# HKU-MedAI/WSI-HGNN

Measured on AMD Instinct MI355X. Metric: edges/s fwd+bwd HEATNet4, 10k-node/6-rel synth graph, 1->8 MI355X, higher is better.
Workload: dtype f32 (fp16x3 emulation: 2-way fp16 split scaled per row (Y = XW^T, dX) or per column (dW), 3 products - bf16x6 for small launches; fp32-class error)

## Files before the change

include/wsi_hgnn.h:

```cpp
#ifndef WSI_HGNN_H
#define WSI_HGNN_H

#include <stdint.h>

#ifdef __cplusplus
extern "C" {
#endif

#define WSI_OK        0
#define WSI_EINVAL  (-22)
#define WSI_ENOSYS  (-38)
#define WSI_EFAULT  (-14)
#define WSI_ENOMEM  (-12)

#define WSI_ABI_VERSION 26

int         wsi_abi_version(void);
const char* wsi_last_error(void);

typedef struct wsi_context wsi_context_t;
int  wsi_context_create(wsi_context_t** out);
void wsi_context_destroy(wsi_context_t* ctx);

#define WSI_ATTN_XCD_CONTIGUOUS 1
// ... 227 lines not shown
int wsi_gate_grad(const float* g, int64_t ldg, const float* a, int64_t lda, const float* b, int64_t ldb,
                  int32_t D, const int32_t* chunk_row, int32_t num_chunks, const int32_t* seg_chunk, int32_t num_segs,
                  const int32_t* seg_gate, const float* skip, int32_t n_gates, float* partial, float* g_skip, void* stream);

int wsi_pool_factors(const float* x, int64_t ldx, int32_t D, const float* w, int64_t ldw, int32_t T, int32_t H, int32_t Bg,
                     const int32_t* chunk_row, int32_t num_chunks, const int32_t* seg_chunk,
                     float* partial, float* hp, float* csum, float* x_mean, void* stream);
int wsi_pool_tmean(const float* tpart, int32_t T, int32_t S, int32_t D, int32_t H, const float* csum, const float* const* bv,
                   const float* scale, float* t_mean, void* stream);
int wsi_pool_bwd_prep(const float* g_pool, int32_t S, int32_t D, int32_t op, const float* counts, const float* z_mean, const float* h_mean,
                      const int32_t* seg_gate, const float* skip, int32_t n_gates, const int32_t* type_gate, int32_t T,
                      float* g_row, float* g_sum, float* g_skip, float* omg, void* stream);
int wsi_pool_bwd_bias(const float* gt_seg, int32_t T, int32_t S, int32_t D, int32_t H, const float* const* bv, const float* csum,
                      float* beta, float* gbv, void* stream);

int wsi_plan_assemble(const int64_t* desc, int32_t nsegs, int32_t total_blocks, void* stream);
int wsi_slot_fill(const int64_t* desc, int32_t nsegs, int32_t total_blocks, void* stream);

int wsi_layernorm_fwd(const float* x, int64_t ldx, int32_t n, int32_t D, float eps,
                      const float* gamma, const float* beta, const int32_t* row_param,
                      float* y, int64_t ldy, float* stats, void* stream);
int wsi_layernorm_bwd(const float* gy, int64_t ldgy, const float* x, int64_t ldx, int32_t n, int32_t D,
                      const float* gamma, const int32_t* row_param, const float* stats,
                      float* gx, int64_t ldgx, float* xhat_gy, int64_t ldp, void* stream);
int wsi_gelu_fwd(const float* x, float* y, int64_t n, void* stream);
int wsi_gelu_bwd(const float* x, const float* gy, float* gx, int64_t n, void* stream);
int wsi_spmm_sum(const float* x, int64_t ldx, int32_t n_out, int32_t D,
                 const int32_t* ptr, const int32_t* idx, const float* edge_w, const float* iscale, const float* oscale,
                 const float* bias, int32_t relu, const float* relu_ref, int64_t ldref,
                 float* out, int64_t ldo, void* stream);
// ... 173 lines not shown
```

wsi-hgnn_amd/csrc/heat_attn.hip:

```cpp
#include "common.h"
#include <math.h>
#include <stdlib.h>
#include <mutex>
#include <type_traits>
#include <new>

namespace wsi {

struct AttnGraph {
    const int32_t* node_seg;
    const int32_t* rowptr;
    const int32_t* src;
    const float* sim;
    const int32_t* order;
    int32_t num_nodes;
    int32_t heavy_n;
    int32_t pass;
    int32_t heavy_deg;
    int32_t xcd;
    uint32_t* absmax;
    const float* score_in;
    const int32_t* gt_row;
};

// ... 432 lines not shown
#pragma unroll
        for (int i = 0; i < V; ++i) {
            float x = 0.f;
#pragma unroll
            for (int pp = 0; pp < kWavesPerBlock; ++pp) x += sm_acc[(pp * V + i) * 64 + lane];
            gqa[i] = x;
        }
    }
    store_vec<V>(gq + (int64_t)w * ldgq + col, gqa);
    if (g.absmax) {
        const uint32_t b = wave_absmax_bits<V>(gqa);
        if (lane == 0) g.absmax[2 * (int64_t)w] = b;
    }
}

template <int V, int LPH, int U, bool POOL = false, bool KONLY = false>
__global__ __launch_bounds__(kBlock) void heat_attn_bwd_p3_kernel(
    const float* __restrict__ qtab, int64_t ldq, const float* __restrict__ g_t, int64_t ldgt,
    const int32_t* __restrict__ colptr, const int32_t* __restrict__ csc_eid, const int32_t* __restrict__ csc_dst,
    const float* __restrict__ inv_rd, const int32_t* __restrict__ order, int32_t num_nodes, int32_t xcd,
    const float* __restrict__ a, const float* __restrict__ gsc,
    float* __restrict__ gk, int64_t ldgk, float* __restrict__ gv, int64_t ldgv, uint32_t* __restrict__ absmax,
    const int32_t* __restrict__ gt_row, AttnPool pool) {
    constexpr int H = 64 / LPH;
    const int lane = threadIdx.x & 63;
    const int blk = xcd ? xcd_remap((int)blockIdx.x, (int)gridDim.x) : (int)blockIdx.x;
    int wave = blk * kWavesPerBlock + (int)(threadIdx.x >> 6);
    wave = __builtin_amdgcn_readfirstlane(wave);
    if (wave >= num_nodes) return;
    int u = order ? order[wave] : wave;
    u = __builtin_amdgcn_readfirstlane(u);
// ... 6 lines not shown
    float cb[POOL ? kPoolTypes : 1];
#pragma unroll
    for (int b = 0; b < (POOL ? kPoolTypes : 1); ++b) cb[b] = 0.f;

    const int j0 = colptr[u], j1 = colptr[u + 1];
    for (int j = j0; j < j1; j += U) {
        float qq[U][V], gt[U][V];
        float aa[U], gg[U];
        int bin[U];
#pragma unroll
        for (int x = 0; x < U; ++x) {
            if (j + x < j1) {
                const int eid = csc_eid[j + x];
                const int w = csc_dst[j + x];
                const int64_t o = (int64_t)eid * H + head;
                if constexpr (!KONLY) aa[x] = a[o] * inv_rd[w];
                gg[x] = gsc[o];
                load_vec<V>(qq[x], qtab + (int64_t)w * ldq + col);
                if constexpr (POOL) bin[x] = pool.ctab_ready ? -1 : pool.row_seg[w] / pool.segs_per_type;
                else if constexpr (!KONLY) load_vec<V>(gt[x], g_t + (int64_t)(gt_row ? gt_row[w] : w) * ldgt + col);
            }
        }
#pragma unroll
        for (int x = 0; x < U; ++x) {
            if (j + x < j1) {
#pragma unroll
                for (int i = 0; i < V; ++i) {
                    gka[i] = fmaf(gg[x], qq[x][i], gka[i]);
                    if constexpr (!POOL && !KONLY) gva[i] = fmaf(aa[x], gt[x][i], gva[i]);
                }
                if constexpr (POOL) {
#pragma unroll
                    for (int b = 0; b < kPoolTypes; ++b) cb[b] += (bin[x] == b) ? aa[x] : 0.f;
                }
            }
        }
    }
    store_vec<V>(gk + (int64_t)u * ldgk + col, gka);
    if constexpr (POOL) {
        const int su = pool.row_seg[u];
        const int tu = su / pool.segs_per_type, gu = su - tu * pool.segs_per_type;
        float racc[V];
        load_vec<V>(racc, pool.g_row + (int64_t)su * (V * 64) + col);
        const float om = pool.omg[tu];
#pragma unroll
        for (int i = 0; i < V; ++i) racc[i] *= om;
        const float* ybase = pool.y + (int64_t)tu * pool.num_segs * H * (V * 64);
#pragma unroll
        for (int b = 0; b < kPoolTypes; ++b) {
            if (b < pool.n_types) {
                if (pool.ctab_ready) cb[b] = pool.ctab[((int64_t)u * pool.n_types + b) * H + head];
                const float* yrow = ybase + (int64_t)(b * pool.segs_per_type + gu) * H * (V * 64) + col;
#pragma unroll
                for (int h = 0; h < H; ++h) {
                    const float c = __shfl(cb[b], h * LPH, 64);
                    float yv[V];
                    load_vec<V>(yv, yrow + h * (V * 64));
#pragma unroll
                    for (int i = 0; i < V; ++i) racc[i] = fmaf(c, yv[i], racc[i]);
                }
                if (!pool.ctab_ready && (lane % LPH) == 0) pool.ctab[((int64_t)u * pool.n_types + b) * H + head] = cb[b];
            }
        }
        store_vec<V>(pool.r_out + (int64_t)u * pool.ldr + col, racc);
        if (absmax) {
            const uint32_t bmax = wave_absmax_bits<V>(gka);
            if (lane == 0) absmax[2 * (int64_t)u + 1] = bmax;
        }
    } else if constexpr (KONLY) {
        if (absmax) {
            const uint32_t b = wave_absmax_bits<V>(gka);
            if (lane == 0) absmax[2 * (int64_t)u + 1] = max(b, absmax[2 * (int64_t)u + 1]);
        }
    } else {
        store_vec<V>(gv + (int64_t)u * ldgv + col, gva);
        if (absmax) {
            const uint32_t b = max(wave_absmax_bits<V>(gka), wave_absmax_bits<V>(gva));
            if (lane == 0) absmax[2 * (int64_t)u + 1] = b;
        }
// ... 538 lines not shown
        if (pflat || srcmajor) {}
        else if (ph) hipLaunchKernelGGL((heat_attn_bwd_p1_kernel<V, LPH, U, false, true>), dim3(blocks), dim3(kBlock), 0, st, tb, gl, g_t, ldgt, score_a, lse, ga, *pool);
        else hipLaunchKernelGGL((heat_attn_bwd_p1_kernel<V, LPH, U>), dim3(blocks), dim3(kBlock), 0, st, tb, gl, g_t, ldgt, score_a, lse, ga, AttnPool{});
        hipLaunchKernelGGL((heat_attn_bwd_p2_kernel<V, LPH, U>), dim3(blocks), dim3(kBlock), 0, st,
                           tb, gl, ew, eb, isd, (const float*)score_a, (const float*)ga, gsc, gea, gq, ldgq);
        hub_join(st, side);
    } else if (blocks > 0) {
        if (pflat || srcmajor) {}
        else if (ph) hipLaunchKernelGGL((heat_attn_bwd_p1_kernel<V, LPH, U, false, true>), dim3(blocks), dim3(kBlock), 0, st,
                                        tb, gd, g_t, ldgt, score_a, lse, ga, *pool);
        else hipLaunchKernelGGL((heat_attn_bwd_p1_kernel<V, LPH, U>), dim3(blocks), dim3(kBlock), 0, st,
                                tb, gd, g_t, ldgt, score_a, lse, ga, AttnPool{});
        hipLaunchKernelGGL((heat_attn_bwd_p2_kernel<V, LPH, U>), dim3(blocks), dim3(kBlock), 0, st,
                           tb, gd, ew, eb, isd, (const float*)score_a, (const float*)ga, gsc, gea, gq, ldgq);
    }
    if (sblocks > 0 && pool)
        hipLaunchKernelGGL((heat_attn_bwd_p3_kernel<V, LPH, U, true>), dim3(sblocks), dim3(kBlock), 0, st,
                           tb.q, tb.ldq, g_t, ldgt, colptr, csc_eid, csc_dst, inv_rd, order_src, num_src, gd.xcd,
                           (const float*)score_a, (const float*)gsc, gk, ldgk, gv, ldgv, gd.absmax, gd.gt_row, *pool);
    else if (sblocks > 0 && srcmajor) {
        constexpr int UC = U;
        auto pass_c = [&](auto uu) {
            hipLaunchKernelGGL((heat_attn_bwd_p3_kernel<V, LPH, decltype(uu)::value, false, true>), dim3(sblocks), dim3(kBlock), 0, st,
                               tb.q, tb.ldq, g_t, ldgt, colptr, csc_eid, csc_dst, inv_rd, order_src, num_src, gd.xcd,
                               (const float*)score_a, (const float*)gsc, gk, ldgk, gv, ldgv, gd.absmax, gd.gt_row, AttnPool{});
        };
#ifdef WSI_ABLATE
        const char* su = knob("WSI_ATTN_SRC_U");
        const int uc = su ? su[su[0] && su[1] ? 1 : 0] - '0' : UC;
        if (uc == 2) pass_c(std::integral_constant<int, 2>{});
        else if (uc == 4) pass_c(std::integral_constant<int, 4>{});
// ... 60 lines not shown
                                 int32_t num_nodes, int32_t num_src, int32_t num_edges, int32_t D, int32_t H,
                                 const int32_t* node_seg, const int32_t* rowptr, const int32_t* src, const float* sim,
                                 const int32_t* colptr, const int32_t* csc_eid, const int32_t* csc_dst,
                                 const float* inv_rd, const int32_t* order_dst, int32_t num_heavy, const int32_t* order_src, int32_t flags,
                                 const float* e_weight, const float* e_bias,
                                 const float* g_t, int64_t ldgt, const int32_t* g_t_row, const float* score, float* score_a, const float* lse,
                                 float* ga, float* gsc, float* gea, float* red_ws,
                                 float* gq, int64_t ldgq, float* gk, int64_t ldgk, float* gv, int64_t ldgv,
                                 float* g_e, uint32_t* g_absmax, const wsi_attn_pool_t* pool, wsi_context_t* ctx, void* stream) {
    if (num_nodes < 0 || num_src < 0 || num_edges < 0 || D <= 0 || H <= 0 || D % H != 0) { set_error("heat_attn_bwd: bad shape"); return WSI_EINVAL; }
    if (!q || !k || (!v && !(pool && (pool->h || pool->gtab))) || !node_seg || !rowptr || !colptr || !inv_rd || !e_weight || !e_bias || !g_t || !score_a ||
        !lse || !ga || !gsc || !gea || !red_ws || !gq || !gk || (!gv && !pool) || !g_e) { set_error("heat_attn_bwd: null pointer"); return WSI_EINVAL; }
    if (reinterpret_cast<uintptr_t>(red_ws) & 7) { set_error("heat_attn_bwd: red_ws must be 8-byte aligned (it holds 512 doubles)"); return WSI_EINVAL; }
    AttnPool ap{};
    if (pool) {
        if (!pool->row_seg || !pool->y || !pool->g_row || !pool->omg || !pool->r_out || !pool->ctab || pool->segs_per_type <= 0 ||
            pool->n_types <= 0 || pool->n_types > kPoolTypes || pool->ldr % 4 != 0 || !aligned16(pool->y) || !aligned16(pool->g_row) ||
            !aligned16(pool->r_out) || num_src != num_nodes) {
            set_error("heat_attn_bwd: bad pool descriptor (1..%d node types, 16-byte aligned tables, num_src == num_nodes)", kPoolTypes);
            return WSI_EINVAL;
        }
        if (pool->h && (!pool->beta || pool->ldh % 4 != 0 || !aligned16(pool->h))) { set_error("heat_attn_bwd: pool.h needs pool.beta and 16-byte aligned rows"); return WSI_EINVAL; }
        ap = AttnPool{pool->row_seg, pool->segs_per_type, pool->n_types, pool->n_types * pool->segs_per_type, pool->y, pool->g_row, pool->omg,
                      pool->r_out, pool->ldr, pool->ctab, pool->ctab_ready, pool->h, pool->ldh, pool->beta, pool->gtab, pool->edge_seg, pool->seg_dst};
        if (pool->gtab && (!pool->edge_seg || !pool->seg_dst)) { set_error("heat_attn_bwd: pool.gtab needs pool.edge_seg and pool.seg_dst"); return WSI_EINVAL; }
    }
    const bool al = (ldq | ldk | (v ? ldv : 0) | ldgt | ldgq | ldgk | (gv ? ldgv : 0)) % 4 == 0 && aligned16(q) && aligned16(k) && aligned16(v) &&
                    aligned16(g_t) && aligned16(gq) && aligned16(gk) && aligned16(gv);
    AttnTables tb{q, ldq, k, ldk, v, ldv};
    if (num_heavy < 0 || num_heavy > num_nodes || (num_heavy > 0 && !order_dst)) { set_error("heat_attn_bwd: bad num_heavy=%d", num_heavy); return WSI_EINVAL; }
    AttnGraph gd{node_seg, rowptr, src, sim, order_dst, num_nodes, num_heavy, 0, heavy_degree(flags), (flags & WSI_ATTN_XCD_CONTIGUOUS) ? 1 : 0, g_absmax, score ? score : score_a, g_t_row};
    const float isd = 1.0f / sqrtf((float)(D / H));
// ... 106 lines not shown
```

wsi-hgnn_amd/csrc/pooled.hip:

```cpp
#include "common.h"
#include <math.h>

namespace wsi {

constexpr int POOL_MAX_TYPES = 16;
struct PtrList { const float* p[POOL_MAX_TYPES]; };

__global__ __launch_bounds__(256) void pool_tmean_kernel(const float* __restrict__ tpart, int tau0, int nt, int T, int S, int D, int H,
                                                         const float* __restrict__ csum, const PtrList bv, const float* __restrict__ scale,
                                                         int accumulate, int finish, float* __restrict__ t_mean) {
    const int s = blockIdx.x, c = blockIdx.y * 256 + threadIdx.x;
    if (c >= D) return;
    const int hh = c / (D / H);
    float acc = accumulate ? t_mean[(int64_t)s * D + c] : 0.f;
    for (int i = 0; i < nt; ++i) {
        const int tau = tau0 + i;
        acc += tpart[((int64_t)tau * S + s) * D + c];
        if (bv.p[i]) acc = fmaf(csum[((int64_t)tau * S + s) * H + hh], bv.p[i][c], acc);
    }
    if (finish && scale) acc *= scale[s];
    t_mean[(int64_t)s * D + c] = acc;
}

__global__ __launch_bounds__(256) void pool_bwd_prep_kernel(const float* __restrict__ g_pool, int S, int D, int mean, const float* __restrict__ counts,
// ... 49 lines not shown
            }
            return;
        }
        blk -= nt * S;
    }
    if (!gbv) return;
    const int tiles = (D + 255) / 256;
    const int i = blk / tiles, c = (blk - i * tiles) * 256 + threadIdx.x, tau = tau0 + i;
    if (i >= nt || c >= D) return;
    const int hh = c / dk;
    float acc = 0.f;
    for (int s = 0; s < S; ++s) acc = fmaf(csum[((int64_t)tau * S + s) * H + hh], gt_seg[(int64_t)s * D + c], acc);
    gbv[(int64_t)tau * D + c] = acc;
}

}

using namespace wsi;

extern "C" int wsi_pool_tmean(const float* tpart, int32_t T, int32_t S, int32_t D, int32_t H, const float* csum, const float* const* bv,
                              const float* scale, float* t_mean, void* stream) {
    if (T <= 0 || S <= 0 || D <= 0 || H <= 0 || D % H) { set_error("pool_tmean: bad argument"); return WSI_EINVAL; }
    if (!tpart || !csum || !bv || !t_mean) { set_error("pool_tmean: null pointer"); return WSI_EINVAL; }
    hipStream_t st = (hipStream_t)stream;
    for (int t0 = 0; t0 < T; t0 += POOL_MAX_TYPES) {
        const int nt = (T - t0 < POOL_MAX_TYPES) ? T - t0 : POOL_MAX_TYPES;
        PtrList L;
        for (int i = 0; i < POOL_MAX_TYPES; ++i) L.p[i] = (i < nt) ? bv[t0 + i] : nullptr;
        hipLaunchKernelGGL(pool_tmean_kernel, dim3(S, (D + 255) / 256), dim3(256), 0, st, tpart, t0, nt, (int)T, (int)S, (int)D, (int)H, csum, L, scale,
                           t0 > 0 ? 1 : 0, t0 + nt >= T ? 1 : 0, t_mean);
// ... 17 lines not shown
                                 float* beta, float* gbv, void* stream) {
    if (T <= 0 || S <= 0 || D <= 0 || H <= 0 || D % H) { set_error("pool_bwd_bias: bad argument"); return WSI_EINVAL; }
    if (!gt_seg || (beta && !bv) || (gbv && !csum)) { set_error("pool_bwd_bias: null pointer"); return WSI_EINVAL; }
    if (!beta && !gbv) return WSI_OK;
    hipStream_t st = (hipStream_t)stream;
    const int tiles = (D + 255) / 256;
    for (int t0 = 0; t0 < T; t0 += POOL_MAX_TYPES) {
        const int nt = (T - t0 < POOL_MAX_TYPES) ? T - t0 : POOL_MAX_TYPES;
        PtrList L;
        for (int i = 0; i < POOL_MAX_TYPES; ++i) L.p[i] = (beta && i < nt) ? bv[t0 + i] : nullptr;
        const int blocks = (beta ? nt * S : 0) + (gbv ? nt * tiles : 0);
        hipLaunchKernelGGL(pool_bwd_bias_kernel, dim3(blocks), dim3(256), 0, st, gt_seg, t0, nt, (int)S, (int)D, (int)H, L, csum, beta, gbv);
    }
    return check_launch("pool_bwd_bias");
}
```

wsi-hgnn_amd/data.py:

```python
from __future__ import annotations

from collections import OrderedDict
from typing import Iterator, List, Optional, Sequence, Tuple

import torch

from . import graph as _graph_mod
from .graph import HeteroGraph, PlanHeader, PlanPieces, _resolve_device, assemble_plan, host_to_device


def augment_draw(seed: int, counter: int, slide: int) -> int:
    from .ops import _fmix32
    return _fmix32(_fmix32(_fmix32(int(seed)) + int(counter) * 0x9E3779B1) + int(slide) * 0x85EBCA6B)


class StoredGraph:

    def __init__(self, g: HeteroGraph, label: int, device: torch.device, resident: bool):
        self.ntypes = g.ntypes
        self.rels = g.canonical_etypes
        self.num_nodes = [g.num_nodes(t) for t in self.ntypes]
        self.label = int(label)
        edges = OrderedDict((r, tuple(x.to(device) for x in g.edges(r))) for r in self.rels)
        sims = {r: g._eframes[r]["sim"].to(device=device, dtype=torch.float32) for r in self.rels}
# ... 468 lines not shown
            sb = self.batch
            return ([[sb.counts[t][b] for t in range(T)] for b in range(B)],
                    [[sb.eoff[(t, b + 1)] - sb.eoff[(t, b)] if b + 1 < B else sb.feb[t] - sb.eoff[(t, b)] for t in range(T)] for b in range(B)])
        n, e = self._counts(self.idxs)
        return [list(x) for x in n], [list(x) for x in e]

    def padded_share(self):
        lay = self.layout
        n, e = self.counts()
        return (lay.N - sum(map(sum, n))) / max(lay.N, 1), (lay.E - sum(map(sum, e))) / max(lay.E, 1)


def _slot_reduce_plan(ops):
    class SlotReducePlan(ops.ReducePlan):

        def has_empty(self) -> bool:
            return True

    return SlotReducePlan
```

wsi-hgnn_amd/ops.py:

```python
from __future__ import annotations

import array
import ctypes
import contextlib
from typing import List, Optional, Sequence, Tuple

import torch

from . import _native as N
from .graph import GraphPlan, SegmentTable, host_to_device



_TIMING = {"on": False, "records": []}


def enable_kernel_timing(on: bool) -> None:
    _TIMING["on"] = bool(on)
    _TIMING["records"] = []


class _Timed:
    def __init__(self, name: str, flops: float = 0.0, mfma_flops: float = 0.0):
        self.name, self.flops, self.mfma_flops = name, flops, mfma_flops
# ... 775 lines not shown
            N.ptr(ew), N.ptr(eb),
            N.ptr(g_t), g_t.shape[1], None, N.ptr(score), N.ptr(a), N.ptr(lse),
            N.ptr(scratch[0]), N.ptr(scratch[1]), N.ptr(scratch[2]), N.ptr(red_ws),
            N.ptr(gkqv, D * 4), ld, N.ptr(gkqv, 0), ld, N.ptr(gkqv, 2 * D * 4), ld,
            N.ptr(g_e), None, None, N.context(), N.stream()), "wsi_heat_attn_bwd")
        return gkqv, g_e[0:1].view(1, 1), g_e[1:2], None, None, None, None


def heat_attention(kqv: torch.Tensor, e_weight: torch.Tensor, e_bias: torch.Tensor, plan: GraphPlan,
                   sim_csr: torch.Tensor, D: int, H: int) -> torch.Tensor:
    return _HeatAttention.apply(kqv, e_weight, e_bias, plan, sim_csr, D, H)


class ReducePlan:

    def __init__(self):
        self.device = None
        self.num_segs = 0
        self.num_chunks = 0
        self.num_rows = 0
        self.first_row = 0
        self.chunk_row = None
        self.chunk_seg = None
        self.seg_chunk = None
        self.ranges: List[Tuple[int, int]] = []
        self._counts = None
        self._inv_counts = None
        self._row_seg = None
        self._nonempty = None
        self._seg_of = {}
# ... 166 lines not shown
        raise ValueError("kqv layout: 'kqv' or 'kvq'")
    _KQV_LAYOUT["order"] = order


def _kqv_blocks(nproj: int):
    return (0, 2, 1) if (nproj == 3 and _KQV_LAYOUT["order"] == "kvq") else (0, 1, 2)


_COLLAPSE_V = {"enabled": True, "min_work": 4.0e9}


def set_value_collapse(on: bool, min_work: Optional[float] = None) -> None:
    _COLLAPSE_V["enabled"] = bool(on)
    if min_work is not None:
        _COLLAPSE_V["min_work"] = float(min_work)


def set_low_rank_readout_grad(on: bool) -> None:
    _LOW_RANK["enabled"] = bool(on)


class _SegmentReduce(torch.autograd.Function):
    @staticmethod
    def forward(ctx, x, rp: ReducePlan, op: int):
        N.require_cuda(x)
        x = x.contiguous()
        out, argmax = _segment_reduce_raw(x, rp, op)
        ctx.rp, ctx.op, ctx.shape = rp, op, x.shape
        ctx.x_id = (x.data_ptr(), x._version)
        ctx.save_for_backward(argmax) if argmax is not None else ctx.save_for_backward(out)
# ... 654 lines not shown
                hit = hctx.cache["gate_of_seg"] = (bc.rp, q @ m.view(T, -1))
            qs = hit[1]
            sig_skip = torch.sigmoid(skip)
            g_skip = (qs @ (bc.g_sum * (bc.x_mean - h_mean)).sum(dim=1)) * (1.0 - sig_skip)
        elif early_gate is not None:
            g_skip = early_gate[0]
        else:
            g_skip = gate_grad_launch(N.stream())[0]
        a = torch.empty_like(score)
        scratch = torch.empty((3, max(E, 1), H), dtype=torch.float32, device=dev)
        red_ws = torch.empty(1024, dtype=torch.float32, device=dev)
        no_v = fwd_factors is not None
        ldp = kqv.shape[1]
        blk = ctx.blk
        kO, qO, vO = blk[0] * D * 4, blk[1] * D * 4, blk[2] * D * 4
        gkqv = torch.empty_like(kqv)
        g_e = torch.empty(2, dtype=torch.float32, device=dev)
        pool_arg = None
        if collapse:
            S, dk = bc.rp.num_segs, D // H
            from .graph import host_to_device
            ytab = torch.empty((T, S, H, D), dtype=torch.float32, device=dev)
            groups = []
            for tau in range(T):
                for hh in range(H):
                    groups.append(dict(A=N.ptr(gt_seg, hh * dk * 4), lda=D, B=N.ptr(P[tau][2], hh * dk * D * 4), ldb=D,
                                       C=N.ptr(ytab, ((tau * S) * H + hh) * D * 4), ldc=H * D, M=S, N=D, K=dk))
            _gemm(N.WSI_GEMM_NN, 0, groups, dev)
            if pre is not None:
                omg = pre[1]
            else:
                qt = hctx.cache.get("gate_of_row_type")
                if qt is None:
                    qt = hctx.cache["gate_of_row_type"] = host_to_device(
                        [[1.0 if (hctx.incoming[i] and hctx.nid[i] == g_) else 0.0 for g_ in range(skip.shape[0])] for i in range(T)], torch.float32, dev).view(T, -1)
                omg = 1.0 - qt @ (sig_skip if sig_skip is not None else torch.sigmoid(skip))
            r_out = torch.empty((n, D), dtype=torch.float32, device=dev)
            bv_ptrs = _ptr_array([P[tau][6] for tau in range(T)])
            gbv = torch.empty((T, D), dtype=torch.float32, device=dev)
            if no_v:
                ctab, hp, csum = fwd_factors
                beta = torch.empty((T, S, H), dtype=torch.float32, device=dev)
                N.check(lib.wsi_pool_bwd_bias(N.ptr(gt_seg), T, S, D, H, bv_ptrs, N.ptr(csum), N.ptr(beta), N.ptr(gbv), N.stream()), "wsi_pool_bwd_bias")
            else:
                ctab = torch.empty((n, T, H), dtype=torch.float32, device=dev)
                beta = None
            gtab = None
            if no_v and T * H <= 32 and T * H * (D + 4) * 4 <= 64 * 1024:
                gtab = torch.empty((n, T, H), dtype=torch.float32, device=dev)
                with _Timed("heat_attn"), _Timed("heat_attn_bwd_pooled"):
                    N.check(lib.wsi_heat_pool_gtab(N.ptr(h), D, D, H, N.ptr(ytab), N.ptr(beta), N.ptr(bc.rp.chunk_row), N.ptr(bc.rp.chunk_seg),
                                                   bc.rp.num_chunks, S // T, T, N.ptr(gtab), N.stream()), "wsi_heat_pool_gtab")
            pool_desc = N.AttnPool(row_seg=N.ptr(bc.rp.row_segment()), segs_per_type=S // T, n_types=T, y=N.ptr(ytab), g_row=N.ptr(bc.g_row),
                                   omg=N.ptr(omg), r_out=N.ptr(r_out), ldr=D, ctab=N.ptr(ctab), ctab_ready=1 if no_v else 0,
                                   h=N.ptr(h) if no_v else None, ldh=D, beta=N.ptr(beta), gtab=N.ptr(gtab),
                                   edge_seg=N.ptr(_edge_segments(plan)) if gtab is not None else None,
                                   seg_dst=N.ptr(_segment_dst(plan)) if gtab is not None else None)
            pool_arg = ctypes.byref(pool_desc)
        _background_flush(dev)
        with _Timed("heat_attn"), _Timed("heat_attn_bwd_pooled" if collapse else "heat_attn_bwd_full"):
            N.check(lib.wsi_heat_attn_bwd(
                N.ptr(kqv, qO), ldp, N.ptr(kqv, kO), ldp, None if no_v else N.ptr(kqv, vO), ldp, n, plan.num_src_rows, E, D, H,
                N.ptr(plan.node_seg), N.ptr(plan.rowptr), N.ptr(plan.src), N.ptr(sim_csr),
                N.ptr(plan.colptr), N.ptr(plan.csc_eid), N.ptr(plan.csc_dst),
                N.ptr(plan.inv_rd), N.ptr(plan.order_dst), plan.num_heavy, N.ptr(plan.order_src), _attn_flags(plan), N.ptr(ew), N.ptr(eb),
                N.ptr(g_t), D, N.ptr(gt_row), N.ptr(score), N.ptr(a), N.ptr(lse), N.ptr(scratch[0]), N.ptr(scratch[1]), N.ptr(scratch[2]), N.ptr(red_ws),
                N.ptr(gkqv, qO), ldp, N.ptr(gkqv, kO), ldp, None if no_v else N.ptr(gkqv, vO), ldp,
                N.ptr(g_e), N.ptr(gkqv_max), pool_arg, N.context(), N.stream()), "wsi_heat_attn_bwd")
        gk_side = _col_stats_side(gkqv, hctx.rows, dev) if (want_col_stats(n, D, D) and (D % 32 == 0)) else None
        g_h = torch.empty((n, D), dtype=torch.float32, device=dev)
        chunked = (D % 32 == 0)
        nproj = 2 if collapse else 3
        gh_cols = ColStats.allocate(hctx.rows, D, dev, sums=True) if (chunked and want_col_stats(n, D, D)) else None
        gh_wrote = True
        if collapse:
            groups = []
            for i, (r0, r1) in enumerate(hctx.rows):
                groups.append(dict(A=N.ptr(gkqv, r0 * ldp * 4), lda=ldp, B=N.ptr(P[i][0]), B1=N.ptr(P[i][1]), b_chunk=D, ldb=D, Bw=[P[i][0], P[i][1]],
                                   C=N.ptr(g_h, r0 * D * 4), ldc=D, R=N.ptr(r_out, r0 * D * 4), ldr=D, M=r1 - r0, N=D, K=2 * D,
                                   **_scale_in(gkqv_max, r0), **_scale_out(gh_max, r0),
                                   **(gh_cols.produce(r0, r1, 0) if gh_cols is not None else {})))
            gh_wrote = _gemm(N.WSI_GEMM_NN, N.WSI_EPI_ADD_R, groups, dev)
        for with_gate in ((True, False) if not collapse else ()):
            idxs = [i for i in range(T) if hctx.incoming[i] == with_gate]
            if not idxs:
                continue
            epi = N.WSI_EPI_ADD_R | (N.WSI_EPI_R_1MG if with_gate else 0)
            if chunked:
                groups = []
                for i in idxs:
# ... 10 lines not shown
                    groups = []
                    for i in idxs:
                        r0, r1 = hctx.rows[i]
                        groups.append(dict(A=N.ptr(gkqv, (r0 * 3 * D + blk[j] * D) * 4), lda=3 * D, B=N.ptr(P[i][j]), ldb=D,
                                           C=N.ptr(g_h, r0 * D * 4), ldc=D, R=N.ptr(g_out, r0 * D * 4), ldr=D,
                                           gate=gate(i) if with_gate else None, M=r1 - r0, N=D, K=D))
                    _gemm(N.WSI_GEMM_NN, epi if j == 0 else N.WSI_EPI_ACCUMULATE, groups, dev)
        wgroups = []
        h_cols = getattr(ctx, "h_cols", None)
        for i, (r0, r1) in enumerate(hctx.rows):
            for j in range(nproj):
                gw = torch.empty_like(P[i][j])
                gb = torch.empty_like(P[i][4 + j])
                grads[8 * i + j] = gw
                grads[8 * i + 4 + j] = gb
                wgroups.append(dict(A=N.ptr(gkqv, (r0 * ldp + blk[j] * D) * 4), lda=ldp, B=N.ptr(h, r0 * D * 4), ldb=D,
                                    C=N.ptr(gw), ldc=D, colsum_out=N.ptr(gb), M=D, N=D, K=r1 - r0,
                                    **(gk_side[0].consume("a", r0, r1, blk[j] * D, want_sums=True) if gk_side is not None else {}),
                                    **(h_cols.consume("b", r0, r1, 0) if h_cols is not None else {})))
        wr = [P[i][k] for i in range(T) for j in range(nproj) for k in (j, 4 + j)]
        keep = [gkqv, h] + ([h_cols.bits] if h_cols is not None else []) + ([gk_side[0].bits, gk_side[0].sums] if gk_side is not None else [])
        outs = [(P[i][k], grads[8 * i + k]) for i in range(T) for j in range(nproj) for k in (j, 4 + j)]
        evs = [gk_side[1]] if gk_side is not None else []
        if not (ctx.background_dw and _background_safe(wr) and _gemm_tn_background(0, wgroups, dev, keep, wr, evs, outs=outs)):
            for ev in evs:
                torch.cuda.current_stream(dev).wait_event(ev)
            _gemm(N.WSI_GEMM_TN, 0, wgroups, dev)
        if collapse:
            if not no_v:
                hp, csum = _pooled_factors(h, ctab, bc.rp, T, H)
                N.check(lib.wsi_pool_bwd_bias(N.ptr(gt_seg), T, S, D, H, None, N.ptr(csum), None, N.ptr(gbv), N.stream()), "wsi_pool_bwd_bias")
# ... 1298 lines not shown
```

Measured before the change: 111.3 million.

## Fold pooled residual into dX GEMM via extended K columns

```diff
diff --git a/include/wsi_hgnn.h b/include/wsi_hgnn.h
--- a/include/wsi_hgnn.h
+++ b/include/wsi_hgnn.h
@@ -265,6 +265,11 @@
 int wsi_pool_bwd_bias(const float* gt_seg, int32_t T, int32_t S, int32_t D, int32_t H, const float* const* bv, const float* csum,
                       float* beta, float* gbv, void* stream);
 
+int32_t wsi_pool_dx_ext_scratch_words(int32_t T);
+int wsi_pool_dx_ext(const float* y, const float* g_row, const float* omg, const float* ctab, const int32_t* row_seg,
+                    const float* const* wk, const float* const* wq, int64_t ldw, int32_t T, int32_t H, int32_t Bg, int32_t D, int32_t n_rows,
+                    uint32_t* scratch, float* yext, float* ext, int64_t ldext, uint32_t* g_absmax, void* stream);
+
 int wsi_plan_assemble(const int64_t* desc, int32_t nsegs, int32_t total_blocks, void* stream);
 int wsi_slot_fill(const int64_t* desc, int32_t nsegs, int32_t total_blocks, void* stream);
 
diff --git a/wsi-hgnn_amd/csrc/heat_attn.hip b/wsi-hgnn_amd/csrc/heat_attn.hip
--- a/wsi-hgnn_amd/csrc/heat_attn.hip
+++ b/wsi-hgnn_amd/csrc/heat_attn.hip
@@ -470,7 +470,7 @@
     }
 }
 
-template <int V, int LPH, int U, bool POOL = false, bool KONLY = false>
+template <int V, int LPH, int U, bool POOL = false, bool KONLY = false, bool NOR = false>
 __global__ __launch_bounds__(kBlock) void heat_attn_bwd_p3_kernel(
     const float* __restrict__ qtab, int64_t ldq, const float* __restrict__ g_t, int64_t ldgt,
     const int32_t* __restrict__ colptr, const int32_t* __restrict__ csc_eid, const int32_t* __restrict__ csc_dst,
@@ -507,7 +507,7 @@
                 const int eid = csc_eid[j + x];
                 const int w = csc_dst[j + x];
                 const int64_t o = (int64_t)eid * H + head;
-                if constexpr (!KONLY) aa[x] = a[o] * inv_rd[w];
+                if constexpr (!KONLY) aa[x] = (NOR && pool.ctab_ready) ? 0.f : a[o] * inv_rd[w];
                 gg[x] = gsc[o];
                 load_vec<V>(qq[x], qtab + (int64_t)w * ldq + col);
                 if constexpr (POOL) bin[x] = pool.ctab_ready ? -1 : pool.row_seg[w] / pool.segs_per_type;
@@ -531,31 +531,37 @@
     }
     store_vec<V>(gk + (int64_t)u * ldgk + col, gka);
     if constexpr (POOL) {
-        const int su = pool.row_seg[u];
-        const int tu = su / pool.segs_per_type, gu = su - tu * pool.segs_per_type;
-        float racc[V];
-        load_vec<V>(racc, pool.g_row + (int64_t)su * (V * 64) + col);
-        const float om = pool.omg[tu];
-#pragma unroll
-        for (int i = 0; i < V; ++i) racc[i] *= om;
-        const float* ybase = pool.y + (int64_t)tu * pool.num_segs * H * (V * 64);
-#pragma unroll
-        for (int b = 0; b < kPoolTypes; ++b) {
-            if (b < pool.n_types) {
-                if (pool.ctab_ready) cb[b] = pool.ctab[((int64_t)u * pool.n_types + b) * H + head];
-                const float* yrow = ybase + (int64_t)(b * pool.segs_per_type + gu) * H * (V * 64) + col;
-#pragma unroll
-                for (int h = 0; h < H; ++h) {
-                    const float c = __shfl(cb[b], h * LPH, 64);
-                    float yv[V];
-                    load_vec<V>(yv, yrow + h * (V * 64));
-#pragma unroll
-                    for (int i = 0; i < V; ++i) racc[i] = fmaf(c, yv[i], racc[i]);
-                }
-                if (!pool.ctab_ready && (lane % LPH) == 0) pool.ctab[((int64_t)u * pool.n_types + b) * H + head] = cb[b];
-            }
-        }
-        store_vec<V>(pool.r_out + (int64_t)u * pool.ldr + col, racc);
+        if constexpr (!NOR) {
+            const int su = pool.row_seg[u];
+            const int tu = su / pool.segs_per_type, gu = su - tu * pool.segs_per_type;
+            float racc[V];
+            load_vec<V>(racc, pool.g_row + (int64_t)su * (V * 64) + col);
+            const float om = pool.omg[tu];
+#pragma unroll
+            for (int i = 0; i < V; ++i) racc[i] *= om;
+            const float* ybase = pool.y + (int64_t)tu * pool.num_segs * H * (V * 64);
+#pragma unroll
+            for (int b = 0; b < kPoolTypes; ++b) {
+                if (b < pool.n_types) {
+                    if (pool.ctab_ready) cb[b] = pool.ctab[((int64_t)u * pool.n_types + b) * H + head];
+                    const float* yrow = ybase + (int64_t)(b * pool.segs_per_type + gu) * H * (V * 64) + col;
+#pragma unroll
+                    for (int h = 0; h < H; ++h) {
+                        const float c = __shfl(cb[b], h * LPH, 64);
+                        float yv[V];
+                        load_vec<V>(yv, yrow + h * (V * 64));
+#pragma unroll
+                        for (int i = 0; i < V; ++i) racc[i] = fmaf(c, yv[i], racc[i]);
+                    }
+                    if (!pool.ctab_ready && (lane % LPH) == 0) pool.ctab[((int64_t)u * pool.n_types + b) * H + head] = cb[b];
+                }
+            }
+            store_vec<V>(pool.r_out + (int64_t)u * pool.ldr + col, racc);
+        } else if (!pool.ctab_ready && (lane % LPH) == 0) {
+#pragma unroll
+            for (int b = 0; b < kPoolTypes; ++b)
+                if (b < pool.n_types) pool.ctab[((int64_t)u * pool.n_types + b) * H + head] = cb[b];
+        }
         if (absmax) {
             const uint32_t bmax = wave_absmax_bits<V>(gka);
             if (lane == 0) absmax[2 * (int64_t)u + 1] = bmax;
@@ -1124,7 +1130,11 @@
         hipLaunchKernelGGL((heat_attn_bwd_p2_kernel<V, LPH, U>), dim3(blocks), dim3(kBlock), 0, st,
                            tb, gd, ew, eb, isd, (const float*)score_a, (const float*)ga, gsc, gea, gq, ldgq);
     }
-    if (sblocks > 0 && pool)
+    if (sblocks > 0 && pool && !pool->r_out)
+        hipLaunchKernelGGL((heat_attn_bwd_p3_kernel<V, LPH, U, true, false, true>), dim3(sblocks), dim3(kBlock), 0, st,
+                           tb.q, tb.ldq, g_t, ldgt, colptr, csc_eid, csc_dst, inv_rd, order_src, num_src, gd.xcd,
+                           (const float*)score_a, (const float*)gsc, gk, ldgk, gv, ldgv, gd.absmax, gd.gt_row, *pool);
+    else if (sblocks > 0 && pool)
         hipLaunchKernelGGL((heat_attn_bwd_p3_kernel<V, LPH, U, true>), dim3(sblocks), dim3(kBlock), 0, st,
                            tb.q, tb.ldq, g_t, ldgt, colptr, csc_eid, csc_dst, inv_rd, order_src, num_src, gd.xcd,
                            (const float*)score_a, (const float*)gsc, gk, ldgk, gv, ldgv, gd.absmax, gd.gt_row, *pool);
@@ -1215,8 +1225,8 @@
     if (reinterpret_cast<uintptr_t>(red_ws) & 7) { set_error("heat_attn_bwd: red_ws must be 8-byte aligned (it holds 512 doubles)"); return WSI_EINVAL; }
     AttnPool ap{};
     if (pool) {
-        if (!pool->row_seg || !pool->y || !pool->g_row || !pool->omg || !pool->r_out || !pool->ctab || pool->segs_per_type <= 0 ||
-            pool->n_types <= 0 || pool->n_types > kPoolTypes || pool->ldr % 4 != 0 || !aligned16(pool->y) || !aligned16(pool->g_row) ||
+        if (!pool->row_seg || !pool->y || !pool->g_row || !pool->omg || !pool->ctab || pool->segs_per_type <= 0 ||
+            pool->n_types <= 0 || pool->n_types > kPoolTypes || (pool->r_out && pool->ldr % 4 != 0) || !aligned16(pool->y) || !aligned16(pool->g_row) ||
             !aligned16(pool->r_out) || num_src != num_nodes) {
             set_error("heat_attn_bwd: bad pool descriptor (1..%d node types, 16-byte aligned tables, num_src == num_nodes)", kPoolTypes);
             return WSI_EINVAL;
diff --git a/wsi-hgnn_amd/csrc/pooled.hip b/wsi-hgnn_amd/csrc/pooled.hip
--- a/wsi-hgnn_amd/csrc/pooled.hip
+++ b/wsi-hgnn_amd/csrc/pooled.hip
@@ -87,6 +87,117 @@
     gbv[(int64_t)tau * D + c] = acc;
 }
 
+constexpr int POOL_EXT = 32;
+constexpr int POOL_EXT_PARTS = 64;
+
+__global__ __launch_bounds__(256) void pool_ext_max_kernel(const PtrList wk, const PtrList wq, int64_t ldw, int vec, const float* __restrict__ y,
+                                                           const float* __restrict__ g_row, const float* __restrict__ omg, int Bg, int S, int H,
+                                                           int D, uint32_t* __restrict__ part) {
+    __shared__ uint32_t red[8];
+    const int tau = blockIdx.y;
+    float mw = 0.f, my = 0.f;
+    auto m4 = [](float m, const float4 v) { return fmaxf(fmaxf(m, fmaxf(fabsf(v.x), fabsf(v.y))), fmaxf(fabsf(v.z), fabsf(v.w))); };
+    const float* yt = y + (int64_t)tau * S * H * D;
+    const int64_t ny = (int64_t)S * H * D, ng = (int64_t)Bg * D;
+    const float om = fabsf(omg[tau]);
+    const float* gr = g_row + (int64_t)tau * Bg * D;
+    const int64_t t0 = (int64_t)blockIdx.x * 256 + threadIdx.x, step = (int64_t)gridDim.x * 256;
+    if (vec) {
+        for (int r = blockIdx.x; r < D; r += gridDim.x)
+            for (int c = 4 * threadIdx.x; c < D; c += 1024) {
+                mw = m4(mw, *reinterpret_cast<const float4*>(wk.p[tau] + (int64_t)r * ldw + c));
+                mw = m4(mw, *reinterpret_cast<const float4*>(wq.p[tau] + (int64_t)r * ldw + c));
+            }
+        for (int64_t e = 4 * t0; e < ny; e += 4 * step) my = m4(my, *reinterpret_cast<const float4*>(yt + e));
+        float mg = 0.f;
+        for (int64_t e = 4 * t0; e < ng; e += 4 * step) mg = m4(mg, *reinterpret_cast<const float4*>(gr + e));
+        my = fmaxf(my, om * mg);
+    } else {
+        for (int r = blockIdx.x; r < D; r += gridDim.x)
+            for (int c = threadIdx.x; c < D; c += 256)
+                mw = fmaxf(mw, fmaxf(fabsf(wk.p[tau][(int64_t)r * ldw + c]), fabsf(wq.p[tau][(int64_t)r * ldw + c])));
+        for (int64_t e = t0; e < ny; e += step) my = fmaxf(my, fabsf(yt[e]));
+        float mg = 0.f;
+        for (int64_t e = t0; e < ng; e += step) mg = fmaxf(mg, fabsf(gr[e]));
+        my = fmaxf(my, om * mg);
+    }
+    uint32_t bw = __float_as_uint(mw), by = __float_as_uint(my);
+#pragma unroll
+    for (int o = 32; o > 0; o >>= 1) {
+        bw = max(bw, (uint32_t)__shfl_xor((int)bw, o, 64));
+        by = max(by, (uint32_t)__shfl_xor((int)by, o, 64));
+    }
+    const int wave = threadIdx.x >> 6;
+    if ((threadIdx.x & 63) == 0) { red[2 * wave] = bw; red[2 * wave + 1] = by; }
+    __syncthreads();
+    if (threadIdx.x < 2) {
+        const int k = threadIdx.x;
+        part[((int64_t)tau * POOL_EXT_PARTS + blockIdx.x) * 2 + k] = max(max(red[k], red[2 + k]), max(red[4 + k], red[6 + k]));
+    }
+}
+
+__device__ __forceinline__ void pool_ext_gammas(const uint32_t* __restrict__ part, int T, int* gam) {
+    for (int t = threadIdx.x; t < T; t += 256) {
+        uint32_t bw = 0u, by = 0u;
+        for (int q = 0; q < POOL_EXT_PARTS; ++q) {
+            bw = max(bw, part[((int64_t)t * POOL_EXT_PARTS + q) * 2]);
+            by = max(by, part[((int64_t)t * POOL_EXT_PARTS + q) * 2 + 1]);
+        }
+        int g = (bw == 0u || by == 0u) ? 0 : (int)((by >> 23) & 0xffu) - (int)((bw >> 23) & 0xffu);
+        gam[t] = g < -96 ? -96 : (g > 96 ? 96 : g);
+    }
+    __syncthreads();
+}
+
+__global__ __launch_bounds__(256) void pool_ext_yext_kernel(const float* __restrict__ y, const float* __restrict__ g_row, const float* __restrict__ omg,
+                                                            const uint32_t* __restrict__ part, int T, int H, int Bg, int D, float* __restrict__ yext) {
+    __shared__ int gam[POOL_MAX_TYPES];
+    pool_ext_gammas(part, T, gam);
+    const int S = T * Bg, J = T * H;
+    const int s = blockIdx.x / POOL_EXT, j = blockIdx.x - s * POOL_EXT;
+    const int tau = s / Bg, g = s - tau * Bg;
+    const int e = -gam[tau];
+    float* out = yext + ((int64_t)s * POOL_EXT + j) * D;
+    if (j < J) {
+        const int b = j / H, h = j - b * H;
+        const float* src = y + (((int64_t)tau * S + b * Bg + g) * H + h) * D;
+        for (int c = threadIdx.x; c < D; c += 256) out[c] = __builtin_ldexpf(src[c], e);
+    } else if (j == J) {
+        const float om = omg[tau];
+        const float* src = g_row + (int64_t)s * D;
+        for (int c = threadIdx.x; c < D; c += 256) out[c] = __builtin_ldexpf(om * src[c], e);
+    } else {
+        for (int c = threadIdx.x; c < D; c += 256) out[c] = 0.f;
+    }
+}
+
+__global__ __launch_bounds__(256) void pool_ext_rows_kernel(const float* __restrict__ ctab, const int32_t* __restrict__ row_seg,
+                                                            const uint32_t* __restrict__ part, int T, int H, int Bg, int n_rows,
+                                                            float* __restrict__ ext, int64_t ldext, uint32_t* __restrict__ absmax) {
+    __shared__ int gam[POOL_MAX_TYPES];
+    pool_ext_gammas(part, T, gam);
+    const int J = T * H;
+    const int u = blockIdx.x * 32 + (threadIdx.x >> 3), c0 = 4 * (threadIdx.x & 7);
+    float v[4] = {0.f, 0.f, 0.f, 0.f};
+    if (u < n_rows) {
+        int tau = row_seg[u] / Bg;
+        tau = tau < 0 ? 0 : (tau >= T ? T - 1 : tau);
+        const int e = gam[tau];
+#pragma unroll
+        for (int i = 0; i < 4; ++i) {
+            const int j = c0 + i;
+            v[i] = __builtin_ldexpf(j < J ? ctab[(int64_t)u * J + j] : (j == J ? 1.f : 0.f), e);
+        }
+        *reinterpret_cast<float4*>(ext + (int64_t)u * ldext + c0) = make_float4(v[0], v[1], v[2], v[3]);
+    }
+    if (absmax) {
+        uint32_t b = __float_as_uint(fmaxf(fmaxf(fabsf(v[0]), fabsf(v[1])), fmaxf(fabsf(v[2]), fabsf(v[3]))));
+#pragma unroll
+        for (int o = 4; o > 0; o >>= 1) b = max(b, (uint32_t)__shfl_xor((int)b, o, 64));
+        if (u < n_rows && (threadIdx.x & 7) == 0) absmax[2 * (int64_t)u + 1] = max(b, absmax[2 * (int64_t)u + 1]);
+    }
+}
+
 }
 
 using namespace wsi;
@@ -134,3 +245,40 @@
     }
     return check_launch("pool_bwd_bias");
 }
+
+extern "C" int32_t wsi_pool_dx_ext_scratch_words(int32_t T) { return T > 0 ? 2 * POOL_EXT_PARTS * T : 0; }
+
+extern "C" int wsi_pool_dx_ext(const float* y, const float* g_row, const float* omg, const float* ctab, const int32_t* row_seg,
+                               const float* const* wk, const float* const* wq, int64_t ldw, int32_t T, int32_t H, int32_t Bg, int32_t D, int32_t n_rows,
+                               uint32_t* scratch, float* yext, float* ext, int64_t ldext, uint32_t* g_absmax, void* stream) {
+    if (T <= 0 || T > POOL_MAX_TYPES || H <= 0 || Bg <= 0 || D <= 0 || n_rows < 0 || T * H + 1 > POOL_EXT) {
+        set_error("pool_dx_ext: bad argument (T * H + 1 <= %d, T <= %d)", POOL_EXT, POOL_MAX_TYPES); return WSI_EINVAL;
+    }
+    if (!scratch || (!yext && !ext)) { set_error("pool_dx_ext: null pointer"); return WSI_EINVAL; }
+    hipStream_t st = (hipStream_t)stream;
+    if (yext) {
+        if (!y || !g_row || !omg || !wk || !wq || ldw < D) { set_error("pool_dx_ext: null pointer or ldw < D"); return WSI_EINVAL; }
+        PtrList K, Q;
+        auto a16 = [](const void* p) { return (reinterpret_cast<uintptr_t>(p) & 15) == 0; };
+        bool vec = D % 4 == 0 && ldw % 4 == 0 && a16(y) && a16(g_row);
+        for (int i = 0; i < POOL_MAX_TYPES; ++i) {
+            K.p[i] = (i < T) ? wk[i] : nullptr;
+            Q.p[i] = (i < T) ? wq[i] : nullptr;
+            if (i < T && (!K.p[i] || !Q.p[i])) { set_error("pool_dx_ext: null weight pointer (type %d)", i); return WSI_EINVAL; }
+            vec = vec && a16(K.p[i]) && a16(Q.p[i]);
+        }
+        const int S = T * Bg;
+        hipLaunchKernelGGL(pool_ext_max_kernel, dim3(POOL_EXT_PARTS, T), dim3(256), 0, st, K, Q, ldw, vec ? 1 : 0, y, g_row, omg, (int)Bg, S, (int)H, (int)D,
+                           scratch);
+        hipLaunchKernelGGL(pool_ext_yext_kernel, dim3(S * POOL_EXT), dim3(256), 0, st, y, g_row, omg, (const uint32_t*)scratch, (int)T, (int)H, (int)Bg,
+                           (int)D, yext);
+    }
+    if (ext && n_rows > 0) {
+        if (!ctab || !row_seg || ldext % 4 != 0 || ldext < POOL_EXT || (reinterpret_cast<uintptr_t>(ext) & 15)) {
+            set_error("pool_dx_ext: null pointer, or extension columns that are not 16-byte aligned rows"); return WSI_EINVAL;
+        }
+        hipLaunchKernelGGL(pool_ext_rows_kernel, dim3((n_rows + 31) / 32), dim3(256), 0, st, ctab, row_seg, (const uint32_t*)scratch, (int)T, (int)H, (int)Bg,
+                           (int)n_rows, ext, ldext, g_absmax);
+    }
+    return check_launch("pool_dx_ext");
+}
diff --git a/wsi-hgnn_amd/data.py b/wsi-hgnn_amd/data.py
--- a/wsi-hgnn_amd/data.py
+++ b/wsi-hgnn_amd/data.py
@@ -506,6 +506,8 @@
 def _slot_reduce_plan(ops):
     class SlotReducePlan(ops.ReducePlan):
 
+        rewritten_in_place = True
+
         def has_empty(self) -> bool:
             return True
 
diff --git a/wsi-hgnn_amd/ops.py b/wsi-hgnn_amd/ops.py
--- a/wsi-hgnn_amd/ops.py
+++ b/wsi-hgnn_amd/ops.py
@@ -813,6 +813,8 @@
 
 class ReducePlan:
 
+    rewritten_in_place = False
+
     def __init__(self):
         self.device = None
         self.num_segs = 0
@@ -1009,6 +1011,88 @@
     _COLLAPSE_V["enabled"] = bool(on)
     if min_work is not None:
         _COLLAPSE_V["min_work"] = float(min_work)
+
+
+_POOL_DX_EXT = {"enabled": True, "launches": 0}
+
+
+def set_pool_dx_extension(on: bool) -> None:
+    _POOL_DX_EXT["enabled"] = bool(on)
+
+
+def _pool_dx_extension_applies(no_v: bool, T: int, H: int, D: int, rp, rows) -> bool:
+    return bool(_POOL_DX_EXT["enabled"] and no_v and T * H + 1 <= 32 and D % 32 == 0 and not rp.rewritten_in_place and rp.segments_of(rows) is not None)
+
+
+def _pool_dx_ext_prepare(gkqv, g_h, Wk, Wq, ytab, g_row, omg, rp, rows, segs, H: int, gkqv_max, gh_max, want_cols: bool) -> dict:
+    lib = N.load()
+    n, ldg = gkqv.shape
+    D, T, S, dev = g_h.shape[1], len(rows), rp.num_segs, gkqv.device
+    yext = torch.empty((S, 32, D), dtype=torch.float32, device=dev)
+    scratch = torch.empty(max(lib.wsi_pool_dx_ext_scratch_words(T), 1), dtype=torch.int32, device=dev)
+    seg_rows = [(a - rp.first_row, b - rp.first_row) for (a, b) in rp.ranges]
+    gh_cols = _segment_col_stats(seg_rows, rows, D, dev) if want_cols else None
+    groups = []
+    for i in range(T):
+        for s_ in range(*segs[i]):
+            r0, r1 = seg_rows[s_]
+            if r1 > r0:
+                groups.append(dict(A=N.ptr(gkqv, r0 * ldg * 4), lda=ldg, B=N.ptr(Wk[i]), B1=N.ptr(Wq[i]), B2=N.ptr(yext, s_ * 32 * D * 4), b_chunk=D, ldb=D,
+                                   C=N.ptr(g_h, r0 * D * 4), ldc=D, M=r1 - r0, N=D, K=2 * D + 32,
+                                   **_scale_in(gkqv_max, r0), **_scale_out(gh_max, r0),
+                                   **(gh_cols.produce(r0, r1, 0) if gh_cols is not None else {})))
+    side = side_stream(dev, "work") if _side_stats_on() else None
+    st = N.stream() if side is None else ctypes.c_void_p(side.cuda_stream)
+    if side is not None:
+        side.wait_stream(torch.cuda.current_stream(dev))
+    N.check(lib.wsi_pool_dx_ext(N.ptr(ytab), N.ptr(g_row), N.ptr(omg), None, None, _ptr_array(Wk), _ptr_array(Wq), D, T, H, S // T, D, n,
+                                N.ptr(scratch), N.ptr(yext), None, 0, None, st), "wsi_pool_dx_ext")
+    keep = [yext, scratch, ytab, g_row, omg]
+    prec = _GEMM_MODES[_PRECISION["mode"]]
+    nbytes = (lib.wsi_gemm_packed_b_bytes(D, 2 * D + 32) + 15) & ~15
+    for i in range(0, len(groups), N.WSI_GEMM_MAX_GROUPS):
+        chunk = groups[i:i + N.WSI_GEMM_MAX_GROUPS]
+        if lib.wsi_gemm_kernel_precision(N.WSI_GEMM_NN, prec, _group_array(chunk), len(chunk)) != N.WSI_GEMM_FP16X3:
+            continue
+        buf = torch.empty(len(chunk) * nbytes // 4, dtype=torch.int32, device=dev)
+        for j, g in enumerate(chunk):
+            g["b_packed"] = N.ptr(buf, j * nbytes)
+        N.check(lib.wsi_gemm_pack_b(N.WSI_GEMM_NN, _group_array(chunk), len(chunk), st), "wsi_gemm_pack_b")
+        keep.append(buf)
+    ev = None
+    if side is not None:
+        ev = torch.cuda.Event()
+        ev.record(side)
+        for t_ in keep + list(Wk) + list(Wq):
+            t_.record_stream(side)
+    return dict(groups=groups, gh_cols=gh_cols, scratch=scratch, event=ev, keep=keep, gkqv=gkqv, gkqv_max=gkqv_max, rp=rp, T=T, H=H, D=D)
+
+
+def _pool_dx_ext_finish(state: dict, ctab):
+    gkqv, rp, T, H, D = state["gkqv"], state["rp"], state["T"], state["H"], state["D"]
+    n, ldg = gkqv.shape
+    dev = gkqv.device
+    if state["event"] is not None:
+        torch.cuda.current_stream(dev).wait_event(state["event"])
+    N.check(N.load().wsi_pool_dx_ext(None, None, None, N.ptr(ctab), N.ptr(rp.row_segment()), None, None, D, T, H, rp.num_segs // T, D, n,
+                                     N.ptr(state["scratch"]), None, N.ptr(gkqv, 2 * D * 4), ldg, N.ptr(state["gkqv_max"]), N.stream()), "wsi_pool_dx_ext")
+    _POOL_DX_EXT["launches"] += 1
+    return state["gh_cols"], _gemm(N.WSI_GEMM_NN, 0, state["groups"], dev)
+
+
+def _pool_dx_ext_project(gkqv, g_h, Wk, Wq, ytab, g_row, omg, ctab, rp, rows, segs, H: int, gkqv_max, gh_max, want_cols: bool):
+    return _pool_dx_ext_finish(_pool_dx_ext_prepare(gkqv, g_h, Wk, Wq, ytab, g_row, omg, rp, rows, segs, H, gkqv_max, gh_max, want_cols), ctab)
+
+
+def _segment_col_stats(seg_rows, type_rows, width: int, device) -> Optional[ColStats]:
+    cs = ColStats.allocate(seg_rows, width, device, sums=True)
+    if cs is None:
+        return None
+    for (r0, r1) in type_rows:
+        inside = [cs.ranges[r] for r in seg_rows if r[1] > r[0] and r0 <= r[0] and r[1] <= r1]
+        if inside:
+            cs.ranges[(r0, r1)] = (inside[0][0], sum(n_ for _, n_ in inside))
+    return cs
 
 
 def set_low_rank_readout_grad(on: bool) -> None:
@@ -1693,7 +1777,9 @@
         ldp = kqv.shape[1]
         blk = ctx.blk
         kO, qO, vO = blk[0] * D * 4, blk[1] * D * 4, blk[2] * D * 4
-        gkqv = torch.empty_like(kqv)
+        ext = collapse and _pool_dx_extension_applies(no_v, T, H, D, bc.rp, hctx.rows)
+        ldg = ldp + 32 if ext else ldp
+        gkqv = torch.empty((n, ldg), dtype=torch.float32, device=dev)
         g_e = torch.empty(2, dtype=torch.float32, device=dev)
         pool_arg = None
         if collapse:
@@ -1714,7 +1800,7 @@
                     qt = hctx.cache["gate_of_row_type"] = host_to_device(
                         [[1.0 if (hctx.incoming[i] and hctx.nid[i] == g_) else 0.0 for g_ in range(skip.shape[0])] for i in range(T)], torch.float32, dev).view(T, -1)
                 omg = 1.0 - qt @ (sig_skip if sig_skip is not None else torch.sigmoid(skip))
-            r_out = torch.empty((n, D), dtype=torch.float32, device=dev)
+            r_out = None if ext else torch.empty((n, D), dtype=torch.float32, device=dev)
             bv_ptrs = _ptr_array([P[tau][6] for tau in range(T)])
             gbv = torch.empty((T, D), dtype=torch.float32, device=dev)
             if no_v:
@@ -1736,6 +1822,11 @@
                                    edge_seg=N.ptr(_edge_segments(plan)) if gtab is not None else None,
                                    seg_dst=N.ptr(_segment_dst(plan)) if gtab is not None else None)
             pool_arg = ctypes.byref(pool_desc)
+        g_h = torch.empty((n, D), dtype=torch.float32, device=dev)
+        ext_state = None
+        if ext:
+            ext_state = _pool_dx_ext_prepare(gkqv, g_h, [P[i][0] for i in range(T)], [P[i][1] for i in range(T)], ytab, bc.g_row, omg, bc.rp, hctx.rows, segs, H,
+                                             gkqv_max, gh_max, want_col_stats(n, D, D))
         _background_flush(dev)
         with _Timed("heat_attn"), _Timed("heat_attn_bwd_pooled" if collapse else "heat_attn_bwd_full"):
             N.check(lib.wsi_heat_attn_bwd(
@@ -1744,15 +1835,16 @@
                 N.ptr(plan.colptr), N.ptr(plan.csc_eid), N.ptr(plan.csc_dst),
                 N.ptr(plan.inv_rd), N.ptr(plan.order_dst), plan.num_heavy, N.ptr(plan.order_src), _attn_flags(plan), N.ptr(ew), N.ptr(eb),
                 N.ptr(g_t), D, N.ptr(gt_row), N.ptr(score), N.ptr(a), N.ptr(lse), N.ptr(scratch[0]), N.ptr(scratch[1]), N.ptr(scratch[2]), N.ptr(red_ws),
-                N.ptr(gkqv, qO), ldp, N.ptr(gkqv, kO), ldp, None if no_v else N.ptr(gkqv, vO), ldp,
+                N.ptr(gkqv, qO), ldg, N.ptr(gkqv, kO), ldg, None if no_v else N.ptr(gkqv, vO), ldg,
                 N.ptr(g_e), N.ptr(gkqv_max), pool_arg, N.context(), N.stream()), "wsi_heat_attn_bwd")
-        gk_side = _col_stats_side(gkqv, hctx.rows, dev) if (want_col_stats(n, D, D) and (D % 32 == 0)) else None
-        g_h = torch.empty((n, D), dtype=torch.float32, device=dev)
+        gk_side = _col_stats_side(gkqv[:, :ldp] if ext else gkqv, hctx.rows, dev) if (want_col_stats(n, D, D) and (D % 32 == 0)) else None
         chunked = (D % 32 == 0)
         nproj = 2 if collapse else 3
-        gh_cols = ColStats.allocate(hctx.rows, D, dev, sums=True) if (chunked and want_col_stats(n, D, D)) else None
+        gh_cols = ColStats.allocate(hctx.rows, D, dev, sums=True) if (chunked and want_col_stats(n, D, D) and not ext) else None
         gh_wrote = True
-        if collapse:
+        if ext:
+            gh_cols, gh_wrote = _pool_dx_ext_finish(ext_state, ctab)
+        elif collapse:
             groups = []
             for i, (r0, r1) in enumerate(hctx.rows):
                 groups.append(dict(A=N.ptr(gkqv, r0 * ldp * 4), lda=ldp, B=N.ptr(P[i][0]), B1=N.ptr(P[i][1]), b_chunk=D, ldb=D, Bw=[P[i][0], P[i][1]],
@@ -1793,7 +1885,7 @@
                 gb = torch.empty_like(P[i][4 + j])
                 grads[8 * i + j] = gw
                 grads[8 * i + 4 + j] = gb
-                wgroups.append(dict(A=N.ptr(gkqv, (r0 * ldp + blk[j] * D) * 4), lda=ldp, B=N.ptr(h, r0 * D * 4), ldb=D,
+                wgroups.append(dict(A=N.ptr(gkqv, (r0 * ldg + blk[j] * D) * 4), lda=ldg, B=N.ptr(h, r0 * D * 4), ldb=D,
                                     C=N.ptr(gw), ldc=D, colsum_out=N.ptr(gb), M=D, N=D, K=r1 - r0,
                                     **(gk_side[0].consume("a", r0, r1, blk[j] * D, want_sums=True) if gk_side is not None else {}),
                                     **(h_cols.consume("b", r0, r1, 0) if h_cols is not None else {})))
```

New measurement: 112.0 million, median of 6. About the same (+0.6%).
